# exoplanet-dev/celerite2

Hardware: AMD Instinct MI355X
Metric: float64 GP log-lik+grad/sec at N=4096 J=8, batched (higher is better)
Workload: dtype f64; 1 GPU; configs[2]: batch of 65536 independent GPs (65536 per GPU), N=4096, J=8 (sum of 4 SHO terms), forward + reverse-mode grad, inputs resident in HBM; global_batch=65536, batch_per_gpu=65536, N=4096, J=8, parallelism=batch-sharded x1, all-gather of log-liks, failed_factorizations=0, clock_prewarm_steps=0

## Files before the change

### celerite2_amd/csrc/c2_dispatch.hpp

```cpp
#pragma once

#define C2_OPTIONS(X)                                                                                                                 \
  X(lanes, "C2_LANES", 0, 's', "lane mapping of the fused log-likelihood kernels: 8 (a group of lanes per series), 4 (four lanes per series, two columns per lane, J = 8), 2 (two lanes per series, J = 8), 1 (one lane per series); unset: by batch size", "profiles/r02_lane_mappings.md") \
  X(lanes1_min_batch_fwd, "C2_LANES1_MIN_BATCH_FWD", 24576, 't', "forward log-likelihood: one lane per series from this many series up (widths 8, 6, 4, 2)", "N = 4096, J = 8: 3.3 vs 4.1 ms at 24576 series, 6.7 vs 10.4 ms at 65536 (profiles/r02_lane_mappings.md)") \
  X(lanes1_min_batch_grad, "C2_LANES1_MIN_BATCH_GRAD", 24576, 't', "log-likelihood + gradient: one lane per series from this many series up (widths 8, 4, 2)", "15.7 vs 16.0 ms at 24576 series, 28.2 vs 41.8 ms at 65536 (profiles/r02_lane_mappings.md)") \
  X(lanes1_min_batch_grad_j6, "C2_LANES1_MIN_BATCH_GRAD_J6", 32768, 't', "the same at width 6 (rows of 48 bytes: no aligned 128-byte runs)", "18.5 vs 20.7 ms at 32768 series, 17.2 vs 15.8 ms at 24576") \
  X(lanes2_min_batch_fwd, "C2_LANES2_MIN_BATCH_FWD", 16385, 't', "forward log-likelihood, J = 8: two lanes per series from this many series up ...", "N = 4096: 2.38 - 2.57 vs 2.25 - 2.43 ms at 16384 series (two columns per lane: one wavefront per SIMD there), 2.59 vs 3.69 at 20480 (one lane), 2.76 vs 3.70 at 24576, 3.37 vs 3.84 at 32768 (profiles/r04_two_lanes.md)") \
  X(lanes2_min_batch_grad, "C2_LANES2_MIN_BATCH_GRAD", 16385, 't', "log-likelihood + gradient, J = 8: two lanes per series from this many series up ...", "11.0 vs 14.6 ms at 18432 series (8 lanes: a third round of wavefronts), 11.4 vs 14.4 at 20480, 12.2 - 12.5 vs 15.2 at 24576; 10.25 vs 10.11 at 16384, 10.17 vs 9.65 at 14336 (8 lanes, reverse sweep by the backward recursion; profiles/r04_two_lanes.md)") \
  X(lanes2_max_batch, "C2_LANES2_MAX_BATCH", 32768, 't', "... up to this many (32 series per wavefront: one wavefront per SIMD)", "14.9 - 16.0 vs 16.2 - 17.2 ms at 32768 series (box to box), 27.5 vs 19.4 at 34816 (profiles/r04_two_lanes.md)") \
  X(loglik_back, "C2_LOGLIK_BACK", 1, 's', "log-likelihood + gradient on the group mappings (up to eight lanes per series): reverse sweep by the BACKWARD recursion from recorded W rows instead of replaying the forward steps; 0 keeps the replay (A/B runs)", "profiles/r04_back8.md") \
  X(lanes4_min_batch, "C2_LANES4_MIN_BATCH", 16384, 't', "forward log-likelihood, J = 8: two columns per lane from this many series up", "14-15 % faster from 16384 series, equal at 8192 (profiles/r01_lanes4.md)") \
  X(lanes4_min_batch_grad, "C2_LANES4_MIN_BATCH_GRAD", 9216, 't', "log-likelihood + gradient, J = 8: four lanes per series (two columns per lane, scaled frame; c2_loglik_q4.hip) from this many series up ...", "N = 4096: 4.99 vs 4.52 ms at 8192 series (8 lanes: one wavefront per SIMD there), 6.10 vs 6.43 at 9216, 6.21 vs 6.60 at 10240, 6.94 vs 7.36 at 12288 (profiles/r05_four_lanes.md)") \
  X(lanes4_max_batch_grad, "C2_LANES4_MAX_BATCH_GRAD", 16384, 't', "... up to this many (one wavefront per SIMD; the two-lane pair takes over beyond)", "8.39 ms at 16384 series against 9.7 on eight lanes at two wavefronts per SIMD (profiles/r05_four_lanes.md)") \
  X(loglik_q4_lines, "C2_LOGLIK_Q4_LINES", 0, 's', "the four-lane gradient pair moves the rows of U, V, bU, bV as aligned 128-byte lines of eight series through LDS tiles (1) or 64 bytes of sixteen series at a time (0); unset: lines from C2_Q4_LINES_MIN_BATCH series", "profiles/r05_four_lanes.md") \
  X(q4_lines_min_batch, "C2_Q4_LINES_MIN_BATCH", 11264, 't', "... that batch size", "N = 4096, lines vs rows: 6.53 vs 6.55 ms at 10240 series, 6.68 vs 6.87 at 12288, 8.20 vs 9.00 at 14336, 8.39 vs 8.96 at 16384; 5.53 vs 5.29 at 8192 (profiles/r05_four_lanes.md)") \
  X(timepar, "C2_TIMEPAR", 0, 's', "forward log-likelihood / factor (widths 4, 2) and the single-rhs solves parallel along TIME: 1 forces, 0 disables; unset: by a cost model (C2_TIMEPAR_ELEMENTS_BIAS) / for small batches of long series", "tools/onepass_grid.py, profiles/r05_onepass.md") \
  X(timepar_min_rows, "C2_TIMEPAR_MIN_ROWS", 1536, 't', "shortest series the time-parallel single-rhs SOLVES take when the batch is not a handful (B * J > 512)", "a handful of series from 384 / 704 / 1024 rows at widths 2 / 4 / 8 (profiles/r02_timepar.md)") \
  X(timepar_max_batch_x_width, "C2_TIMEPAR_MAX_BATCH_X_WIDTH", 8192, 't', "largest B * J the time-parallel single-rhs solves take", "linear in the batch beyond one wavefront per SIMD (profiles/r02_timepar.md)") \
  X(timepar_elements_bias, "C2_TIMEPAR_ELEMENTS_BIAS", 100, 't', "forward log-likelihood (widths 8, 4, 2) and factor (widths 4, 2): the time-parallel forms on chunk elements are taken when their modelled time x this / 100 is below the row-by-row kernel's (the model: use_timepar in c2_loglik.hip; 50 favours them, 200 the row-by-row kernels)", "width 4, 1024 series: log-likelihood 0.044 ms up to 1024 rows, 0.109 at 4096 (row by row 0.22 us per row); factor 0.09 / 0.25 ms; 4096 x 4096: 0.38 vs 0.88 and 0.82 vs 1.02 ms; 8192 x 1024: 0.28 vs 0.24 (tools/onepass_grid.py, profiles/r05_onepass.md)") \
  X(timepar_grad, "C2_TIMEPAR_GRAD", 0, 's', "log-likelihood GRADIENT (and factor_rev) parallel along time, widths 1 .. 8: 1 forces, 0 disables; unset: small batches of long series", "tools/timepar_grad_time.py, profiles/r02_timepar_grad.md") \
  X(timepar_grad_min_rows, "C2_TIMEPAR_GRAD_MIN_ROWS", 1024, 't', "shortest series the time-parallel gradient takes at widths 7, 8 beyond a handful of series (768 at widths 3 .. 6, 512 at 1, 2; 256 for at most 4096 chunks)", "one series draws level at ~400 / ~600 / ~800 rows at J = 2 / 4, 6 / 8 (tools/timepar_grad_time.py)") \
  X(timepar_grad_min_rows_handful, "C2_TIMEPAR_GRAD_MIN_ROWS_HANDFUL", 384, 't', "shortest series the time-parallel gradient takes for a handful of series (at most 4096 chunks of 64 rows; they run with 16-row chunks)", "round 5 (the row-by-row pair in the scaled frame), one series, J = 8: 0.336 vs 0.276 ms row by row at 256 rows, 0.381 vs 0.376 at 384, 0.430 vs 0.476 at 512, 0.87 vs 3.25 at 4096 (tools/crossovers.py)") \
  X(timepar_grad_max_chunks, "C2_TIMEPAR_GRAD_MAX_CHUNKS", 32768, 't', "largest number of 64-row chunks (B * ceil(N / 64)) the time-parallel gradient takes", "1024 x 4096 at J = 4: 3.6 vs 3.0 ms row by row") \
  X(timepar_cond_limit, "C2_TIMEPAR_COND_LIMIT", 0, 't', "if > 0: largest conditioning kappa = max a_n / d_n for which the result of the time-parallel gradient stands; beyond it the row-by-row kernels recompute the batch behind the device-side gate (0, the default: no limit)", "rounding moves ANY float64 evaluation by c eps kappa^2 of the largest gradient entry: the oracle itself c = 0.4 (against its own extended-precision evaluation), the row-by-row kernels ~0.05, the time-parallel form ~0.01 and 0.6 in the worst draw of 9000 -- typically the closer of the two to the oracle, hence no limit by default (tools/kappa_sweep.py, tools/verify_words.py, profiles/r03_timepar_verification.md)") \
  X(verify_fallback, "C2_VERIFY_FALLBACK", 1, 's', "0 (diagnostics only): keep the result of a time-parallel form whatever its device-side verification says", "tools/verify_words.py") \
  X(factor_iter, "C2_FACTOR_ITER", 0, 's', "factor by Newton iterations on the chunk start states: 1 forces, 0 disables; unset: from 2048 rows and at most 32768 chunks (widths 4, 2: from 32768 / 131072 rows)", "tools/factor_iter_time.py: 4096 rows 1.21 -> 0.76 ms, 1e5 rows 29.5 -> 1.0 ms at J = 8") \
  X(factor_scan8, "C2_FACTOR_SCAN8", 1, 's', "width 8: the chunk start states of that form EXACT from the scanned chunk elements (up-sweep + down-sweep of the tree, then ONE pass) instead of Newton iterations on them; 0: the iterations", "tools/kernel_breakdown.sh factor 1 4096 8: eight iterations 513 us (profiles/r06_scan8.md)") \
  X(tpg_rows, "C2_TPG_ROWS", 0, 's', "chunk length of the time-parallel gradient / Newton factor / chunk-map solves: 16, 32 or 64; unset: 16 up to 4096 rows and 32 beyond for at most 4096 chunks of 64 rows, else 64 (the log-likelihood gradient: 32 up to 9216 chunks of 64 rows)", "one series of 4096 rows 1.33 -> 1.03 -> 0.73 ms (64 -> 32 -> 16 rows), 1e5 rows 1.68 -> 1.25 ms with 32") \
  X(tpg_rows16_max_rows, "C2_TPG_ROWS16_MAX_ROWS", 4096, 't', "longest series that takes 16-row chunks", "chains of more than 256 chunks cost accuracy first (9000 rows: 1.3e-11 vs 4e-12), then time") \
  X(dropin_long_rows, "C2_DROPIN_LONG_ROWS", 512, 't', "shortest series factor + S and factor_rev take in their time-parallel form (at least 128)", "tools/bench_ops.py, J = 8: factor_rev 1 x 512 0.38 -> 0.15 ms, 512 x 4096 3.0 -> 1.6 ms") \
  X(long_min_rows, "C2_LONG_MIN_ROWS", 512, 't', "shortest series the chunk-map solves (with F / several right-hand sides) and the long-series reverse sweeps take (at least 128)", "1 x 4096 + F 0.60 -> 0.06 ms, 64 x 1024 0.13 -> 0.05 ms (tools/bench_ops.py)") \
  X(rev_long, "C2_REV_LONG", 0, 's', "the four reverse sweeps as opposite sweep + per-row pass: 1 forces, 0 disables; unset: small batches of long series", "one series of 1e5 rows, J = 8: solve_lower_rev 18.3 -> 0.15 ms (profiles/r02_long_series_rocprof.md)") \
  X(scan_min_rows, "C2_SCAN_MIN_ROWS", 1024, 't', "shortest series the chunked products (c2_scan.hip) take on batches of at most 128 series (at least 256)", "1 x 4096 0.60 -> 0.08 ms, 64 x 4096 0.63 -> 0.15 ms; 1024 x 2048 would lose (0.36 -> 1.01 ms)") \
  X(scan_min_chunk, "C2_SCAN_MIN_CHUNK", 0, 's', "chunk length of the chunked products (at least 64); unset: the power of two next to 0.5 sqrt(N)", "one series, J = 8: 20000 rows 0.79 -> 0.16 ms, 1e5 rows 0.80 -> 0.32 ms") \
  X(solve_chunk_col_ms, "C2_SOLVE_CHUNK_COL_MS", 0.05, 't', "cost model of the chunk-map solves: fixed cost (ms) of one right-hand side", "64 x 4096: 0.07 ms, 512 x 4096: 0.24 ms (tools/bench_ops.py)") \
  X(solve_chunk_ms, "C2_SOLVE_CHUNK_MS", 6e-6, 't', "... cost (ms) per 64-row chunk and right-hand side", "same measurement") \
  X(solve_row_us, "C2_SOLVE_ROW_US", 0.15, 't', "... against the row-by-row sweep: microseconds per row whatever the batch", "4096 rows: 0.63 ms with one right-hand side") \
  X(solve_row_rhs_us, "C2_SOLVE_ROW_RHS_US", 0.025, 't', "... plus microseconds per row and right-hand side", "4096 rows: 1.29 ms with 8 right-hand sides") \
  X(sweep_cols, "C2_SWEEP_COLS", 1, 's', "0: forward sweeps with 9 .. 32 right-hand sides at J = 8 (no workspace) on the lanes-over-rhs kernel (16 / 32 lanes per series) instead of eight lanes per series with several columns per lane and Y / Z in groups of four rows; 2: the second column slice of a reverse sweep with 17 .. 24 right-hand sides keeps two columns per lane instead of one (A/B runs)", "B = 8192, N = 4096: profiles/r04_nrhs_scan.md; one column per lane for the narrow slice: solve_lower_rev at 17 / 20 / 24 right-hand sides 25.2 / 23.5 / 23.5 -> 20.0 / 20.9 / 20.4 ms (profiles/r05_nrhs_scan.md)") \
  X(solve_cols, "C2_SOLVE_COLS", 0, 's', "solve_lower / solve_upper without workspace as chunk maps with lanes over the right-hand sides (every column in the same three launches; J <= 16): 1 forces, 0 disables; unset: 16 and more right-hand sides on small batches, by the cost model of solve_cols_shape", "1 x 4096 with 1024 right-hand sides: profiles/r04_large_nrhs.md") \
  X(solve_cols_min_rows, "C2_SOLVE_COLS_MIN_ROWS", 512, 't', "shortest series that form takes", "below, a launch is a few hundred steps of 0.26 us: nothing to gain behind three launches") \
  X(mfma, "C2_MFMA", 1, 's', "0: long-series products (J = 16; 16 / 32 / 64 right-hand sides) on the VALU instead of the fp64 matrix cores", "N = 1e7: 3.1 vs 9.2 ms (profiles/r02_ubench_memory_and_mfma.md)") \
  X(kernel_values_tile, "C2_KERNEL_VALUES_TILE", 1, 's', "0: c2_kernel_values with a thread (an exponential and a sincos) per entry instead of 32 x 64 tiles with one sincos per tile row / column and angle addition", "64 x 4096 x 256, four complex terms: 1.04 ms per entry (profiles/r06_predict.md)") \
// ... 49 lines not shown
```

### celerite2_amd/csrc/c2_loglik.hip

```cpp
#include <cstdint>
#include <cstdlib>
#include <type_traits>

#include "c2_loglik_helpers.hpp"
#include "../../include/celerite2_amd.h"
#include "c2_internal.hpp"
#include "c2_launch.hpp"

#ifdef C2_REV_TIMING
__device__ unsigned long long c2_dbg[8];
extern "C" void c2_internal_read_dbg(unsigned long long *out) {
  hipMemcpyFromSymbol(out, HIP_SYMBOL(c2_dbg), sizeof(unsigned long long) * 8);
  unsigned long long z[8] = {0};
  hipMemcpyToSymbol(HIP_SYMBOL(c2_dbg), z, sizeof(z));
}
#endif

namespace c2 {

template <int G>
struct Ckpt {
  static constexpr int W = G + 4;
};

template <int G>
__device__ __forceinline__ void fwd_chain(double p, double u, double v, double an, double yn, const double (&pX)[G],
                                          const double (&uX)[G], double (&SX)[G], double &F, double &w, double &d,
                                          double &z, double &rd, double *xslot, int lane, double *tau_out = nullptr) {
  double wX[G];
  xgather_dpp<G>(w, xslot, lane, wX);
  const double dw = d * w;
  double tau0 = 0.0, tau1 = 0.0;
#pragma unroll
  for (int k = 0; k < G; ++k) {
    const double s = (pX[k] * p) * fma(dw, wX[k], SX[k]);
    SX[k] = s;
    if (k & 1) tau1 = fma(uX[k], s, tau1);
    else tau0 = fma(uX[k], s, tau0);
  }
  const double tau = tau0 + tau1;
  if (tau_out) *tau_out = tau;
  F = p * fma(w, z, F);
  double rd_ = tau * u, rz_ = u * F;
  gsum2<G>(rd_, rz_);
  const double dn = an - rd_;
  const double zn = yn - rz_;
  rd = rcp_nr(dn);
  w = (v - tau) * rd;
  d = dn;
  z = zn;
}

#ifndef C2_FWD_RING
#define C2_FWD_RING 8
#endif
#ifndef C2_FWD_OCC
#define C2_FWD_OCC 1
#endif
#ifndef C2_REV_OCC
#define C2_REV_OCC 1
#endif
#ifndef C2_REV_APARK
#define C2_REV_APARK 1
#endif
template <int G>
struct SymPack {
  static constexpr int PER_STEP = kWave + (G - 1) * (kWave / 2);
  static __device__ __forceinline__ int off(int l, int k) {
    const int b = 31 - __builtin_clz(k), hb = 1 << b;
    const int o = (l & hb) ? (l ^ k) : l;
    const int idx = ((o >> (b + 1)) << b) | (o & (hb - 1));
    return kWave + (k - 1) * (kWave / 2) + idx;
  }
};

// ... 127 lines not shown
  if (b < B) {
    const double xm = fmax(fabs(x[b * x_bs]), fabs(x[b * x_bs + N - 1]));
    for (int k = 0; k < T.Jc; ++k) fast = fast && (fabs(T.dc[(T.batched ? b * T.Jc : 0) + k]) * xm < kSincosFastMax);
  }
  double m = 0.0;
  if (words && (int)threadIdx.x < wpg && wpg * g + threadIdx.x < nwaves) {
    m = __longlong_as_double((long long)words[2 * (wpg * g + threadIdx.x) + 1]);
    if (m != m) m = __builtin_inf();
  }
#pragma unroll
  for (int sft = 1; sft < kWave; sft <<= 1) m = fmax(m, __shfl_xor(m, sft, kWave));
  if (!__all(fast)) m = __builtin_inf();
  if (threadIdx.x == 0) {
    const unsigned long long bits = (unsigned long long)__double_as_longlong(m);
    gate[g] = bits;
    atomicMax(head, bits);
    if (!(m <= kBackwardGuard)) atomicAdd(head + 1, 1ull);
  }
}

template <int G, int R, int C, int MODE, bool PAD, int OCC = C2_FWD_OCC, bool TT = false>
__global__ __launch_bounds__(kWave, OCC) void k_loglik_fwd(int64_t B, int64_t N, int Jrt, const double *__restrict__ t,
                                                         int64_t t_bs, const double *__restrict__ c, int64_t c_bs,
                                                         const double *__restrict__ a,
                                                         const double *__restrict__ U,
                                                         const double *__restrict__ V,
                                                         const double *__restrict__ y, double *__restrict__ ll,
                                                         int32_t *__restrict__ flag, double *__restrict__ ckpt,
                                                         int64_t nseg, double *__restrict__ Wst,
                                                         double2 *__restrict__ DZst,
                                                         const unsigned long long *__restrict__ gate,
                                                         const unsigned long long *__restrict__ segguard = nullptr,
                                                         TermsArgs8 T8 = TermsArgs8{},
                                                         const unsigned long long *__restrict__ tgate = nullptr) {
  if (gate_closed(gate, (int64_t)blockIdx.x * (kWave / G))) return;
  static_assert(!TT || (G >= 2 && G <= 8 && !PAD && MODE != 2), "coefficient-level form: full groups of two to eight lanes");
  if constexpr (TT) { if (!tt_group_open(tgate, (int64_t)blockIdx.x * (kWave / G))) return; }
  constexpr bool CKPT = MODE == 1, FACTOR = MODE == 2, REC = MODE != 0;
  static_assert(!CKPT || R % C == 0, "block length must be a multiple of the checkpoint interval");
  constexpr int SPW = kWave / G;
  constexpr int NV = (R + G - 1) / G;
  __shared__ __attribute__((aligned(16))) double xs[3][kWave];
  __shared__ __attribute__((aligned(16))) double sin_[2][3][SPW][R];
  __shared__ __attribute__((aligned(16))) double2 sout[SPW][R];
  const int J = PAD ? Jrt : G;
  const Geo<G> L(B, J);
  const int lane = L.lane, j = L.j, grp = L.lane / G;
  const bool act = PAD ? L.act : true;
  const int64_t ot = (int64_t)L.sl * t_bs, on = (int64_t)L.sl * N, oj = (int64_t)L.sl * N * J + L.jj;
  const double *tb = t + L.b0 * t_bs + ot, *ab = a + L.b0 * N + on, *yb = y + L.b0 * N + on;
  const double *Ub = U + L.b0 * N * J + oj, *Vb = V + L.b0 * N * J + oj;
  const double cj = act ? c[L.b * c_bs + j] : 0.0;
  LaneTerm lt;
  if constexpr (TT) lt.load(T8, L.b, j, G);
  double *ckw = CKPT ? ckpt + (size_t)blockIdx.x * (nseg + (segguard != nullptr ? 1 : 0)) * CkptRec<G>::DOUBLES : nullptr;
  int soff[G];
  soff[0] = lane;
#pragma unroll
  for (int k = 1; k < G; ++k) soff[k] = SymPack<G>::off(lane, k);
  const bool wrec = CKPT && Wst != nullptr;
  double *wst = FACTOR ? Wst + L.b0 * N * J + oj : nullptr;
  double *wrp = wrec ? Wst + (size_t)blockIdx.x * N * kWave + lane : nullptr;
  double2 *dzst = CKPT ? DZst + L.b0 * N + on : nullptr;
  double *dst = FACTOR ? reinterpret_cast<double *>(DZst) + L.b0 * N + on : nullptr;
  const bool stw = PAD ? (L.valid && act) : true;

  double SX[G];
#pragma unroll
  for (int k = 0; k < G; ++k) SX[k] = 0.0;
  double d = 1.0;
  double rd = 1.0;
  double w = 0.0;
  double z = 0.0;
  double F = 0.0;
  double prod = 1.0;
  int eacc = 0;
  double quad = 0.0;
  int32_t fl = 0;

  double vt[NV], va[NV], vy[NV];
  auto vload = [&](int64_t nb) {
#pragma unroll
    for (int m = 0; m < NV; ++m) {
      int64_t row = nb + m * G + j;
      row = (row < N) ? row : N - 1;
      vt[m] = tb[row]; va[m] = ab[row]; vy[m] = yb[row];
    }
  };
  auto vstage = [&](int q) {
#pragma unroll
    for (int m = 0; m < NV; ++m) {
      const int idx = m * G + j;
      if (G * NV == R || idx < R) {
        sin_[q][0][grp][idx] = vt[m]; sin_[q][1][grp][idx] = va[m]; sin_[q][2][grp][idx] = vy[m];
      }
    }
  };
  vload(0); vstage(0);
  vload(R); vstage(1);
  vload(2 * R);

  constexpr int RR = R < C2_FWD_RING ? R : C2_FWD_RING;
  double ru[RR], rv[RR];
  const double *up = Ub, *vp = Vb;
  auto load_row = [&](int r, int ahead, int64_t n, bool clamp) {
    if constexpr (!TT) {
      int64_t o = ahead;
      if (clamp && n >= N) o -= n - (N - 1);
      ru[r] = act ? up[o * J] : 0.0; rv[r] = act ? vp[o * J] : 0.0;
    }
  };
#pragma unroll
  for (int r = 0; r < RR; ++r) load_row(r, r, r, true);

  const bool sparse = wrec && !(__longlong_as_double((long long)segguard[2 * blockIdx.x]) > kBackwardGuard);
  lds_order();
  double tnext = sin_[0][0][grp][0];
  double pc = 1.0, uc = ru[0];
  double vcur = 0.0;
  if constexpr (TT) lt.uv(tnext, uc, vcur);
  double pXc[G], uXc[G];
  xs[0][lane] = pc; xs[1][lane] = uc;
  lds_order();
  xgather_lds<G>(xs[0], lane, pXc);
  xgather_lds<G>(xs[1], lane, uXc);
  lds_order();

  auto block = [&](int64_t n0, int q, auto checked_tag) {
    constexpr bool CHECKED = decltype(checked_tag)::value;
#pragma unroll
    for (int r = 0; r < R; ++r) {
      const int64_t n = n0 + r;
      if (!CHECKED || n < N) {
        if (CKPT && (r % C == 1 % C)) {
          const int64_t m = (n - 1) / C;
          if (!sparse || (m % kAnchor == 0 && m > 0))
            ckpt_store<G>(ckw + m * CkptRec<G>::DOUBLES, lane, soff, SX, F, w);
        }
        const double tn = tnext, yn = sin_[q][2][grp][r];
        const double an = TT ? sin_[q][1][grp][r] + lt.A0 : sin_[q][1][grp][r];
        const double tn1 = (r + 1 < R) ? sin_[q][0][grp][r + 1] : sin_[q ^ 1][0][grp][0];
        const int rn = (r + 1) % R;
        double v, un1;
        if constexpr (TT) {
          v = vcur;
          lt.uv(tn1, un1, vcur);
        } else {
          v = rv[r % RR]; un1 = ru[rn % RR];
        }
        const double pn1 = exp_decay(cj * (tn - tn1));
        double pXn[G], uXn[G];
        xs[0][lane] = pn1; xs[1][lane] = un1;
        lds_order();
        xgather_lds<G>(xs[0], lane, pXn);
        xgather_lds<G>(xs[1], lane, uXn);
        lds_order();
        fwd_chain<G>(pc, uc, v, an, yn, pXc, uXc, SX, F, w, d, z, rd, xs[2], lane);
        if (REC) {
          if (FACTOR && stw && (((fl == 0) & (d > 0.0)) | (n == 0))) wst[n * J] = w;
          if (CKPT && wrec) wrp[(size_t)n * kWave] = w;
          sout[grp][r] = make_double2(d, z);
        }
        load_row(r % RR, r + RR, n + RR, CHECKED);
        fl = ((fl == 0) & (d <= 0.0)) ? (int32_t)n : fl;
        prod *= d;
        quad = fma(z * z, rd, quad);
        if (r % 2 == 1 || r == R - 1) {
          int e;
          prod = frexp(prod, &e);
          eacc += e;
        }
        tnext = tn1;
        pc = pn1; uc = un1;
#pragma unroll
        for (int k = 0; k < G; ++k) { pXc[k] = pXn[k]; uXc[k] = uXn[k]; }
      }
    }
    lds_order();
    if (REC) {
#pragma unroll
      for (int m = 0; m < NV; ++m) {
        const int idx = m * G + j;
        if ((G * NV == R || idx < R) && (!CHECKED || n0 + idx < N)) {
          if (CKPT) dzst[n0 + idx] = sout[grp][idx];
          else if (fl == 0 || n0 + idx <= fl) dst[n0 + idx] = sout[grp][idx].x;
        }
      }
    }
    vstage(q);
    vload(n0 + 3 * R);
    lds_order();
  };
  int64_t n0 = 0;
  int q = 0;
  auto advance = [&]() { up += R * J; vp += R * J; q ^= 1; };
  for (; n0 + 2 * R <= N; n0 += R) { block(n0, q, std::false_type{}); advance(); }
  for (; n0 < N; n0 += R) { block(n0, q, std::true_type{}); advance(); }

  if (wrec) ckpt_store<G>(ckw + nseg * CkptRec<G>::DOUBLES, lane, soff, SX, F, w);
  if (L.valid && j == 0) {
    flag[L.b] = fl;
    if (!FACTOR) {
      int e;
      prod = frexp(prod, &e);
      const double logdet = log(prod) + (double)(eacc + e) * kLn2;
      ll[L.b] = fl ? -INFINITY : -0.5 * (logdet + (double)N * kLog2Pi) - 0.5 * quad;
    }
  }
}

__device__ __forceinline__ void apark(double x, int &lo, int &hi) {
  asm("v_accvgpr_write_b32 %0, %1" : "=a"(lo) : "v"(__double2loint(x)));
  asm("v_accvgpr_write_b32 %0, %1" : "=a"(hi) : "v"(__double2hiint(x)));
}
__device__ __forceinline__ double afetch(int lo, int hi) {
  int l, h;
  asm("v_accvgpr_read_b32 %0, %1" : "=v"(l) : "a"(lo));
  asm("v_accvgpr_read_b32 %0, %1" : "=v"(h) : "a"(hi));
  return __hiloint2double(h, l);
}

template <int G, int C, bool PAD, bool FR, bool BACK = false, int OCC = C2_REV_OCC, bool TT = false>
__global__ __launch_bounds__(kWave, OCC) void k_loglik_rev(int64_t B, int64_t N, int Jrt, const double *__restrict__ t,
                                                         int64_t t_bs, const double *__restrict__ c, int64_t c_bs,
                                                         const double *__restrict__ U,
                                                         const double *__restrict__ V,
                                                         const double2 *__restrict__ DZst,
                                                         const double *__restrict__ ckpt, int64_t nseg,
                                                         const int32_t *__restrict__ flag, double *__restrict__ bt,
                                                         double *__restrict__ bc, double *__restrict__ ba,
                                                         double *__restrict__ bU, double *__restrict__ bV,
// ... 70 lines not shown
  const double wD = (TT && !lt.re && !lt.odd) ? lt.D : 0.0;
  int vAlo[TT ? C : 1], vAhi[TT ? C : 1];

  int soff[G];
  soff[0] = lane;
#pragma unroll
  for (int k = 1; k < G; ++k) soff[k] = SymPack<G>::off(lane, k);

  double MX[G];
#pragma unroll
  for (int k = 0; k < G; ++k) MX[k] = 0.0;
  double bF = 0.0, carry = 0.0, bcj = 0.0;
  double bVn = 0.0, ban = 0.0, bzn = 0.0;

  double vt[NV];
  double2 vdz[NV];
  double iu[C], iw[C], ibw[FR ? C : 1];
  double cS[G], cF = 0.0, cW = 0.0, tck = 0.0;
  auto load_segment = [&](int64_t k) {
    const int64_t n_lo = 1 + k * C;
    const bool full = n_lo + C <= N;
#pragma unroll
    for (int m = 0; m < NV; ++m) {
      int64_t row = n_lo - 1 + m * G + j;
      row = (row < N) ? row : N - 1;
      vt[m] = tb[row];
      if constexpr (FR) vdz[m] = make_double2(fdb[row], fbdb[row]);
      else vdz[m] = dzb[row];
    }
#pragma unroll
    for (int r = 0; r < C; ++r) {
      const int64_t n = (full || n_lo + r < N) ? n_lo + r : N - 1;
      if constexpr (!TT) iu[r] = act ? Ub[n * J] : 0.0;
      if constexpr (BACK) iw[r] = V[((size_t)blockIdx.x * N + (n - 1)) * kWave + lane];
      else iw[r] = act ? Vb[(n - 1) * J] : 0.0;
      if constexpr (FR) ibw[r] = act ? fbWb[(n - 1) * J] : 0.0;
    }
    if constexpr (FR) {
      const int64_t m = n_lo - 1;
#pragma unroll
      for (int kk = 0; kk < G; ++kk) {
        const int i = j ^ kk;
        cS[kk] = (m >= 1 && act && i < J) ? Scol[m * J * J + i] : 0.0;
      }
      tck = tb[m >= 1 ? m - 1 : 0];
    } else if constexpr (BACK) {
      if ((k + 1) % astep == 0 || k == nseg - 1)
        ckpt_load<G>(ckw + (k + 1) * CkptRec<G>::DOUBLES, lane, soff, cS, cF, cW);
    } else {
      ckpt_load<G>(ckw + k * CkptRec<G>::DOUBLES, lane, soff, cS, cF, cW);
    }
  };

  double carT = tb[N - 1];
  double2 carDZ = FR ? make_double2(fdb[N - 1], fbdb[N - 1]) : dzb[N - 1];
  double carR = rcp_nr(carDZ.x);
  const double wlast = (FR && act) ? Vb[(N - 1) * J] : 0.0, bwlast = (FR && act) ? fbWb[(N - 1) * J] : 0.0;
  if (nseg > 0) load_segment(nseg - 1);
#ifdef C2_REV_TIMING
  unsigned long long tacc[5] = {0, 0, 0, 0, 0}, tlast = 0;
#define C2_TCK(i) do { const unsigned long long tn_ = __builtin_readcyclecounter(); if (i) tacc[i] += tn_ - tlast; tlast = tn_; } while (0)
#else
#define C2_TCK(i)
#endif

  double carS[BACK ? G : 1], carF = 0.0;
  double tref = 0.0, gtop = 1.0, igtop = 1.0;
#pragma unroll
  for (int i = 0; i < (BACK ? G : 1); ++i) carS[i] = 0.0;
// ... 409 lines not shown
    const int JC = T8.Jc, JR = G - 2 * JC;
    const double bcp = dpp_mov<kDppXor1>(bcj);
    if (lt.re) { G8.bar[L.b * JR + j] = sba + accA; G8.bcr[L.b * JR + j] = bcj; }
    else if (!lt.odd) {
      const int64_t o = L.b * JC + ((j - JR) >> 1);
      G8.bac[o] = sba + accA; G8.bbc[o] = accB; G8.bdc[o] = accD; G8.bcc[o] = bcj + bcp;
    }
  } else if (st) { bVb[0] = BACK ? bVn * gtop : bVn; bUb[0] = 0.0; bc[L.b * J + j] = bcj; }
}

}

using namespace c2;

#ifndef C2_CKPT_C
#define C2_CKPT_C 8
#endif
#ifndef C2_FWD_R
#define C2_FWD_R C2_CKPT_C
#endif
#ifndef C2_FWD_R8
#define C2_FWD_R8 16
#endif

static int64_t simd_count();
namespace {
template <int MODE>
int launch_fwd(int64_t B, int64_t N, int64_t J, const double *t, int64_t t_bs, const double *c, int64_t c_bs,
               const double *a, const double *U, const double *V, const double *y, double *ll, int32_t *flag,
               double *ckpt, int64_t nseg, double *Wst, double2 *DZst, hipStream_t s,
               const unsigned long long *gate = nullptr, const unsigned long long *segguard = nullptr, bool occ2 = false) {
  const int G_ = group_size(J);
  const dim3 grid((unsigned)((B * G_ + kWave - 1) / kWave));
  if (MODE == 1 && occ2 && J == 8) {
    hipLaunchKernelGGL((k_loglik_fwd<8, C2_FWD_R8, C2_CKPT_C, (MODE == 1 ? 1 : 0), false, 2>), grid, dim3(kWave), 0, s, B, N, (int)J, t, t_bs, c,
                       c_bs, a, U, V, y, ll, flag, ckpt, nseg, Wst, DZst, gate, segguard);
    return launch_ok();
  }
#define C2_FWD(G, R, C)                                                                                          \
  do {                                                                                                           \
    if (J == G)                                                                                                  \
      hipLaunchKernelGGL((k_loglik_fwd<G, R, C, MODE, false>), grid, dim3(kWave), 0, s, B, N, (int)J, t, t_bs,   \
                         c, c_bs, a, U, V, y, ll, flag, ckpt, nseg, Wst, DZst, gate, segguard);                 \
    else                                                                                                         \
      hipLaunchKernelGGL((k_loglik_fwd<G, R, C, MODE, true>), grid, dim3(kWave), 0, s, B, N, (int)J, t, t_bs,    \
                         c, c_bs, a, U, V, y, ll, flag, ckpt, nseg, Wst, DZst, gate, segguard);                 \
  } while (0)
  switch (G_) {
    case 1: C2_FWD(1, C2_FWD_R, C2_CKPT_C); break;
    case 2: C2_FWD(2, C2_FWD_R, C2_CKPT_C); break;
    case 4: C2_FWD(4, C2_FWD_R, C2_CKPT_C); break;
    case 8: C2_FWD(8, C2_FWD_R8, C2_CKPT_C); break;
    case 16: C2_FWD(16, 8, 4); break;
    default: C2_FWD(32, 4, 2); break;
  }
#undef C2_FWD
  return launch_ok();
}
}

static bool use_lanes4(int64_t B, int64_t J, bool grad) {
  if (J != 8) return false;
  const int forced = opt::has(opt::k_lanes) ? (int)opt::ival(opt::k_lanes) : 0;
  if (forced == 4) return true;
  if (forced == 8 || forced == 1 || forced == 2) return false;
  if (grad) return B >= opt::ival(opt::k_lanes4_min_batch_grad) && B <= opt::ival(opt::k_lanes4_max_batch_grad);
  return B >= opt::ival(opt::k_lanes4_min_batch);
}

static size_t lanes1_gate_words(int64_t B) { return (size_t)((kGateHeadWords + (B + kWave - 1) / kWave + 1) & ~(int64_t)1); }
static bool use_lanes2(int64_t B, int64_t N, int64_t J, bool grad) {
  if (!c2_internal_loglik_k2_ok(B, N, J)) return false;
  const int forced = opt::has(opt::k_lanes) ? (int)opt::ival(opt::k_lanes) : 0;
  if (forced) return forced == 2;
  return B <= opt::ival(opt::k_lanes2_max_batch) &&
         B >= opt::ival(grad ? opt::k_lanes2_min_batch_grad : opt::k_lanes2_min_batch_fwd);
}
static size_t lanes1_record_doubles(int64_t B, int64_t N, int64_t J) {
  return J == 8 ? c2_internal_loglik_t_record_doubles8(B, N)
// ... 153 lines not shown
      rc = keep_first(rc, hipFreeAsync(tmp, s));
      return rc;
    }
    (void)hipGetLastError();
  }
  if (capturing == hipStreamCaptureStatusNone && use_timepar(B, N, J, true)) {
    const size_t nd = c2_internal_loglik_timepar_doubles(B, N, J);
    void *tmp = nullptr;
    if (nd > 0 && c2::temp_alloc(&tmp, (nd + 2) * sizeof(double), s) == hipSuccess) {
      unsigned long long *guard = (unsigned long long *)tmp;
      int rc = c2_internal_loglik_timepar(B, N, J, t, t_bs, c, c_bs, a, U, V, y, ll, flag, (double *)tmp + 2, guard, stream);
      if (rc == C2_OK)
        rc = launch_fwd<0>(B, N, J, t, t_bs, c, c_bs, a, U, V, y, ll, flag, nullptr, 0, nullptr, nullptr, s, guard + 1);
      rc = keep_first(rc, hipFreeAsync(tmp, s));
      return rc;
    }
    (void)hipGetLastError();
  }
  return launch_fwd<0>(B, N, J, t, t_bs, c, c_bs, a, U, V, y, ll, flag, nullptr, 0, nullptr, nullptr, s);
}

static inline int ckpt_interval(int G_) { return G_ <= 8 ? C2_CKPT_C : (G_ == 16 ? 4 : 2); }

struct GradWs {
  size_t ck, w, dz, guard, total;
};
static inline GradWs grad_ws(int64_t B, int64_t N, int64_t J, bool back = false) {
  const int G_ = group_size(J), C_ = ckpt_interval(G_);
  const int64_t nseg = (N - 1 + C_ - 1) / C_;
  GradWs g;
  const size_t waves = ((size_t)B * G_ + kWave - 1) / kWave;
  g.ck = waves * (size_t)(nseg + (back ? 1 : 0)) * ((size_t)kWave + (size_t)(G_ - 1) * (kWave / 2) + 2 * kWave);
  g.ck = (g.ck + 1) & ~(size_t)1;
  g.w = back ? waves * (size_t)N * kWave : 0;
  g.dz = (size_t)B * N * 2;
  g.guard = back ? 2 * waves : 0;
  g.total = g.ck + g.w + g.dz + g.guard;
  return g;
}
static int64_t simd_count() {
  static int64_t n = 0;
  if (n == 0) {
    int dev = 0, cus = 0;
    if (hipGetDevice(&dev) != hipSuccess || hipDeviceGetAttribute(&cus, hipDeviceAttributeMultiprocessorCount, dev) != hipSuccess || cus <= 0)
      cus = 256;
    n = 4 * (int64_t)cus;
  }
  return n;
}
static bool use_back(int64_t N, int64_t J) {
  if (opt::off(opt::k_loglik_back)) return false;
  return group_size(J) <= 8 && N >= 2;
}

size_t c2_internal_factor_scratch_doubles(int64_t B, int64_t N, int64_t J) {
  const size_t n1 = c2_internal_factor_iter_doubles(B, N, J), n2 = c2_internal_timepar_doubles(B, N, J) + 2;
  return ((n1 > n2 ? n1 : n2) + 1) & ~(size_t)1;
}
int c2_internal_factor_fused_ws(int64_t B, int64_t N, int64_t J, const double *t, int64_t t_bs, const double *c,
                                int64_t c_bs, const double *a, const double *U, const double *V, double *d, double *W,
                                int32_t *flag, int allow_timepar, double *scratch, c2_stream_t stream) {
  hipStream_t s = (hipStream_t)stream;
  hipStreamCaptureStatus capturing = hipStreamCaptureStatusNone;
  (void)hipStreamIsCapturing(s, &capturing);
  const bool may_alloc = capturing == hipStreamCaptureStatusNone;
  auto room = [&](size_t nd, void **tmp) {
    if (scratch) { *tmp = scratch; return true; }
// ... 299 lines not shown
}

size_t c2_internal_loglik_g8_tt_doubles(int64_t B, int64_t N, int64_t J) { return grad_ws(B, N, J, true).total; }
int c2_internal_loglik_g8_tt_ok(int64_t B, int64_t N, int64_t J) {
  return (J == 8 || J == 4 || J == 2) && N >= 2 && B >= 1 && (B * J + kWave - 1) / kWave <= simd_count();
}
int c2_internal_loglik_g8_tt_grad(int64_t B, int64_t N, int64_t J, int64_t Jc, int coef_batched, const double *ar, const double *ac,
                                  const double *bc, const double *dc, const double *c, const double *x, int64_t x_bs,
                                  const double *diag, const double *y, double *ll, double *bar, double *bcr, double *bac,
                                  double *bbc, double *bcc, double *bdc, double *bx, double *bdiag, double *by,
                                  int32_t *flag, double *work, unsigned long long *guard, c2_stream_t stream) {
  if (Jc < 0 || 2 * Jc > J || !c2_internal_loglik_g8_tt_ok(B, N, J)) return C2_ERR_UNSUPPORTED;
  hipStream_t s = (hipStream_t)stream;
  constexpr int C_ = C2_CKPT_C;
  const int64_t nseg = (N - 1 + C_ - 1) / C_;
  const GradWs ws = grad_ws(B, N, J, true);
  double *ckpt = work, *Wrec = ckpt + ws.ck;
  double2 *DZst = reinterpret_cast<double2 *>(ckpt + ws.ck + ws.w);
  unsigned long long *segg = reinterpret_cast<unsigned long long *>(ckpt + ws.ck + ws.w + ws.dz);
  const dim3 grid((unsigned)((B * J + kWave - 1) / kWave));
  const TermsArgs8 T{ar, ac, bc, dc, coef_batched, (int)Jc};
  const TermsGrads8 G{bar, bcr, bac, bbc, bcc, bdc};
  unsigned long long *tgate = guard + kGateHeadWords;
  hipLaunchKernelGGL(k_anchor_spans, grid, dim3(256), 0, s, B, N, (int)J, C_, kWave / (int)J, x, x_bs, c, J, segg);
  if (int e = launch_ok()) return e;
  if (int e = hip_check(hipMemsetAsync(guard, 0, 8 * kGateHeadWords, s))) return e;
  hipLaunchKernelGGL(k_tt8_gate, dim3((unsigned)((B + 63) / 64)), dim3(kWave), 0, s, B, N, (int64_t)grid.x, (int)J,
                     (const unsigned long long *)segg, T, x, x_bs, guard, tgate);
  if (int e = launch_ok()) return e;
#define C2_TTG(G_, R_)                                                                                                                \
  do {                                                                                                                                \
    hipLaunchKernelGGL((k_loglik_fwd<G_, R_, C2_CKPT_C, 1, false, 1, true>), grid, dim3(kWave), 0, s, B, N, G_, x, x_bs, \
                       c, J, diag, (const double *)nullptr, (const double *)nullptr, y, ll, flag, ckpt, nseg, Wrec, DZst,             \
                       (const unsigned long long *)nullptr, (const unsigned long long *)segg, T, (const unsigned long long *)tgate);  \
    if (int e = launch_ok()) return e;                                                                                                \
    hipLaunchKernelGGL((k_loglik_rev<G_, C2_CKPT_C, false, false, true, 1, true>), grid, dim3(kWave), 0, s, B, N, G_, x,  \
                       x_bs, c, J, (const double *)nullptr, (const double *)Wrec, (const double2 *)DZst, (const double *)ckpt, nseg,  \
                       (const int32_t *)flag, bx, (double *)nullptr, bdiag, (double *)nullptr, (double *)nullptr, by,                 \
                       (const double *)nullptr, (const double *)nullptr, (const double *)nullptr,                                     \
                       (const unsigned long long *)nullptr, (const unsigned long long *)segg, T, G, (const unsigned long long *)tgate); \
  } while (0)
  if (J == 8) C2_TTG(8, C2_FWD_R8);
  else if (J == 4) C2_TTG(4, C2_FWD_R);
  else C2_TTG(2, C2_FWD_R);
#undef C2_TTG
  return launch_ok();
}
int c2_internal_loglik_g8_tt(int64_t B, int64_t N, int64_t J, int64_t Jc, int coef_batched, const double *ar, const double *ac,
                             const double *bc, const double *dc, const double *c, const double *x, int64_t x_bs,
                             const double *diag, const double *y, double *ll, int32_t *flag, unsigned long long *guard,
                             c2_stream_t stream) {
  if (!(J == 8 || J == 4 || J == 2) || Jc < 0 || 2 * Jc > J || B < 1 || N < 1) return C2_ERR_UNSUPPORTED;
  hipStream_t s = (hipStream_t)stream;
  const dim3 grid((unsigned)((B * J + kWave - 1) / kWave));
  const TermsArgs8 T{ar, ac, bc, dc, coef_batched, (int)Jc};
  unsigned long long *tgate = guard + kGateHeadWords;
  if (int e = hip_check(hipMemsetAsync(guard, 0, 8 * kGateHeadWords, s))) return e;
  hipLaunchKernelGGL(k_tt8_gate, dim3((unsigned)((B + 63) / 64)), dim3(kWave), 0, s, B, N, (int64_t)grid.x, (int)J,
                     (const unsigned long long *)nullptr, T, x, x_bs, guard, tgate);
  if (int e = launch_ok()) return e;
#define C2_TTF(G_, R_)                                                                                                                \
  hipLaunchKernelGGL((k_loglik_fwd<G_, R_, C2_CKPT_C, 0, false, 1, true>), grid, dim3(kWave), 0, s, B, N, G_, x, x_bs, c, \
                     J, diag, (const double *)nullptr, (const double *)nullptr, y, ll, flag, (double *)nullptr, (int64_t)0,           \
                     (double *)nullptr, (double2 *)nullptr, (const unsigned long long *)nullptr, (const unsigned long long *)nullptr, \
                     T, (const unsigned long long *)tgate)
  if (J == 8) C2_TTF(8, C2_FWD_R8);
  else if (J == 4) C2_TTF(4, C2_FWD_R);
// ... 43 lines not shown
```

Measured before the change: 2.374 million GP/s.

## Run eight-lane gradient forward pass in scaled frame between anchors, record W in pairs

Inside the backward guard, the forward log-likelihood pass on the group lane mappings now works in a frame rescaled at periodic anchors. This drops the per-row decay product and its LDS gather and exchange, and replaces them with one scaling factor gathered through DPP. The recorded W rows are also stored and read as double2 pairs, which halves the number of record transactions in both the forward and the reverse kernels. The cost is extra rescaling at anchors and a new numerical path that can be switched off with an option. The one-lane mapping selected at this batch size may not go through this kernel.

```diff
diff --git a/celerite2_amd/csrc/c2_dispatch.hpp b/celerite2_amd/csrc/c2_dispatch.hpp
--- a/celerite2_amd/csrc/c2_dispatch.hpp
+++ b/celerite2_amd/csrc/c2_dispatch.hpp
@@ -9,6 +9,7 @@
   X(lanes2_min_batch_grad, "C2_LANES2_MIN_BATCH_GRAD", 16385, 't', "log-likelihood + gradient, J = 8: two lanes per series from this many series up ...", "11.0 vs 14.6 ms at 18432 series (8 lanes: a third round of wavefronts), 11.4 vs 14.4 at 20480, 12.2 - 12.5 vs 15.2 at 24576; 10.25 vs 10.11 at 16384, 10.17 vs 9.65 at 14336 (8 lanes, reverse sweep by the backward recursion; profiles/r04_two_lanes.md)") \
   X(lanes2_max_batch, "C2_LANES2_MAX_BATCH", 32768, 't', "... up to this many (32 series per wavefront: one wavefront per SIMD)", "14.9 - 16.0 vs 16.2 - 17.2 ms at 32768 series (box to box), 27.5 vs 19.4 at 34816 (profiles/r04_two_lanes.md)") \
   X(loglik_back, "C2_LOGLIK_BACK", 1, 's', "log-likelihood + gradient on the group mappings (up to eight lanes per series): reverse sweep by the BACKWARD recursion from recorded W rows instead of replaying the forward steps; 0 keeps the replay (A/B runs)", "profiles/r04_back8.md") \
+  X(loglik_fwd_scaled, "C2_LOGLIK_FWD_SCALED", 1, 't', "log-likelihood + gradient on the group mappings (up to eight lanes per series): 1 (the default), the forward pass of a wavefront within the backward guard runs in the scaled frame between anchors (no decay products per row); 0 keeps the unscaled loop for every wavefront (A/B runs; both sides in tests/test_gpu_eight_lane_frame.py)", "profiles/eight_lane_forward_frame.md") \
   X(lanes4_min_batch, "C2_LANES4_MIN_BATCH", 16384, 't', "forward log-likelihood, J = 8: two columns per lane from this many series up", "14-15 % faster from 16384 series, equal at 8192 (profiles/r01_lanes4.md)") \
   X(lanes4_min_batch_grad, "C2_LANES4_MIN_BATCH_GRAD", 9216, 't', "log-likelihood + gradient, J = 8: four lanes per series (two columns per lane, scaled frame; c2_loglik_q4.hip) from this many series up ...", "N = 4096: 4.99 vs 4.52 ms at 8192 series (8 lanes: one wavefront per SIMD there), 6.10 vs 6.43 at 9216, 6.21 vs 6.60 at 10240, 6.94 vs 7.36 at 12288 (profiles/r05_four_lanes.md)") \
   X(lanes4_max_batch_grad, "C2_LANES4_MAX_BATCH_GRAD", 16384, 't', "... up to this many (one wavefront per SIMD; the two-lane pair takes over beyond)", "8.39 ms at 16384 series against 9.7 on eight lanes at two wavefronts per SIMD (profiles/r05_four_lanes.md)") \
diff --git a/celerite2_amd/csrc/c2_loglik.hip b/celerite2_amd/csrc/c2_loglik.hip
--- a/celerite2_amd/csrc/c2_loglik.hip
+++ b/celerite2_amd/csrc/c2_loglik.hip
@@ -41,6 +41,33 @@
   const double tau = tau0 + tau1;
   if (tau_out) *tau_out = tau;
   F = p * fma(w, z, F);
+  double rd_ = tau * u, rz_ = u * F;
+  gsum2<G>(rd_, rz_);
+  const double dn = an - rd_;
+  const double zn = yn - rz_;
+  rd = rcp_nr(dn);
+  w = (v - tau) * rd;
+  d = dn;
+  z = zn;
+}
+
+template <int G>
+__device__ __forceinline__ void fwd_chain_scaled(double u, double v, double an, double yn, const double (&uX)[G],
+                                                 double (&SX)[G], double &F, double &w, double &d, double &z, double &rd,
+                                                 double *xslot, int lane) {
+  double wX[G];
+  xgather_dpp<G>(w, xslot, lane, wX);
+  const double dw = d * w;
+  double tau0 = 0.0, tau1 = 0.0;
+#pragma unroll
+  for (int k = 0; k < G; ++k) {
+    const double s = fma(dw, wX[k], SX[k]);
+    SX[k] = s;
+    if (k & 1) tau1 = fma(uX[k], s, tau1);
+    else tau0 = fma(uX[k], s, tau0);
+  }
+  const double tau = tau0 + tau1;
+  F = fma(w, z, F);
   double rd_ = tau * u, rz_ = u * F;
   gsum2<G>(rd_, rz_);
   const double dn = an - rd_;
@@ -234,7 +261,8 @@
                                                          const unsigned long long *__restrict__ gate,
                                                          const unsigned long long *__restrict__ segguard = nullptr,
                                                          TermsArgs8 T8 = TermsArgs8{},
-                                                         const unsigned long long *__restrict__ tgate = nullptr) {
+                                                         const unsigned long long *__restrict__ tgate = nullptr,
+                                                         int fscaled = 1) {
   if (gate_closed(gate, (int64_t)blockIdx.x * (kWave / G))) return;
   static_assert(!TT || (G >= 2 && G <= 8 && !PAD && MODE != 2), "coefficient-level form: full groups of two to eight lanes");
   if constexpr (TT) { if (!tt_group_open(tgate, (int64_t)blockIdx.x * (kWave / G))) return; }
@@ -262,7 +290,9 @@
   for (int k = 1; k < G; ++k) soff[k] = SymPack<G>::off(lane, k);
   const bool wrec = CKPT && Wst != nullptr;
   double *wst = FACTOR ? Wst + L.b0 * N * J + oj : nullptr;
-  double *wrp = wrec ? Wst + (size_t)blockIdx.x * N * kWave + lane : nullptr;
+  static_assert(!CKPT || R % 2 == 0, "rows are recorded in pairs: a block starts at an even row");
+  double2 *wrp = wrec ? reinterpret_cast<double2 *>(Wst) + (size_t)blockIdx.x * ((N + 1) >> 1) * kWave + lane : nullptr;
+  double whold = 0.0;
   double2 *dzst = CKPT ? DZst + L.b0 * N + on : nullptr;
   double *dst = FACTOR ? reinterpret_cast<double *>(DZst) + L.b0 * N + on : nullptr;
   const bool stw = PAD ? (L.valid && act) : true;
@@ -316,6 +346,9 @@
   for (int r = 0; r < RR; ++r) load_row(r, r, r, true);
 
   const bool sparse = wrec && !(__longlong_as_double((long long)segguard[2 * blockIdx.x]) > kBackwardGuard);
+  constexpr bool FRAME = CKPT && G <= 8 && OCC == 1;
+  const bool scaled = FRAME && sparse && fscaled != 0;
+  double tref = 0.0, gc = 1.0, igc = 1.0;
   lds_order();
   double tnext = sin_[0][0][grp][0];
   double pc = 1.0, uc = ru[0];
@@ -328,8 +361,9 @@
   xgather_lds<G>(xs[1], lane, uXc);
   lds_order();
 
-  auto block = [&](int64_t n0, int q, auto checked_tag) {
+  auto block = [&](int64_t n0, int q, auto checked_tag, auto scaled_tag) {
     constexpr bool CHECKED = decltype(checked_tag)::value;
+    constexpr bool SC = decltype(scaled_tag)::value;
 #pragma unroll
     for (int r = 0; r < R; ++r) {
       const int64_t n = n0 + r;
@@ -350,17 +384,41 @@
         } else {
           v = rv[r % RR]; un1 = ru[rn % RR];
         }
-        const double pn1 = exp_decay(cj * (tn - tn1));
-        double pXn[G], uXn[G];
-        xs[0][lane] = pn1; xs[1][lane] = un1;
-        lds_order();
-        xgather_lds<G>(xs[0], lane, pXn);
-        xgather_lds<G>(xs[1], lane, uXn);
-        lds_order();
-        fwd_chain<G>(pc, uc, v, an, yn, pXc, uXc, SX, F, w, d, z, rd, xs[2], lane);
+        double pn1 = 1.0, gn1 = 1.0, ign1 = 1.0, wout;
+        double pXn[SC ? 1 : G], uXn[G];
+        if constexpr (SC) {
+          const bool anchor = (r % C == 0) && n > 0 && (n / C) % kAnchor == 0;
+          if (anchor) tref = tn;
+          gn1 = exp_decay(cj * (tref - tn1));
+          ign1 = rcp_nr(gn1);
+          un1 *= gn1;
+          xgather_dpp<G>(un1, xs[1], lane, uXn);
+          fwd_chain_scaled<G>(uc, v * igc, an, yn, uXc, SX, F, w, d, z, rd, xs[2], lane);
+          wout = w * gc;
+          if (anchor) {
+            double gX[G];
+            xgather_dpp<G>(gc, xs[2], lane, gX);
+#pragma unroll
+            for (int k = 0; k < G; ++k) SX[k] *= gX[k] * gc;
+            F *= gc;
+            w = wout;
+          }
+        } else {
+          pn1 = exp_decay(cj * (tn - tn1));
+          xs[0][lane] = pn1; xs[1][lane] = un1;
+          lds_order();
+          xgather_lds<G>(xs[0], lane, pXn);
+          xgather_lds<G>(xs[1], lane, uXn);
+          lds_order();
+          fwd_chain<G>(pc, uc, v, an, yn, pXc, uXc, SX, F, w, d, z, rd, xs[2], lane);
+          wout = w;
+        }
         if (REC) {
           if (FACTOR && stw && (((fl == 0) & (d > 0.0)) | (n == 0))) wst[n * J] = w;
-          if (CKPT && wrec) wrp[(size_t)n * kWave] = w;
+          if (CKPT && wrec) {
+            if (r % 2 == 0) whold = wout;
+            else wrp[(size_t)(n >> 1) * kWave] = make_double2(whold, wout);
+          }
           sout[grp][r] = make_double2(d, z);
         }
         load_row(r % RR, r + RR, n + RR, CHECKED);
@@ -374,8 +432,14 @@
         }
         tnext = tn1;
         pc = pn1; uc = un1;
-#pragma unroll
-        for (int k = 0; k < G; ++k) { pXc[k] = pXn[k]; uXc[k] = uXn[k]; }
+        if constexpr (SC) {
+          gc = gn1; igc = ign1;
+#pragma unroll
+          for (int k = 0; k < G; ++k) uXc[k] = uXn[k];
+        } else {
+#pragma unroll
+          for (int k = 0; k < G; ++k) { pXc[k] = pXn[k]; uXc[k] = uXn[k]; }
+        }
       }
     }
     lds_order();
@@ -396,9 +460,23 @@
   int64_t n0 = 0;
   int q = 0;
   auto advance = [&]() { up += R * J; vp += R * J; q ^= 1; };
-  for (; n0 + 2 * R <= N; n0 += R) { block(n0, q, std::false_type{}); advance(); }
-  for (; n0 < N; n0 += R) { block(n0, q, std::true_type{}); advance(); }
-
+  if constexpr (FRAME) {
+    if (scaled) {
+      tref = tnext;
+      for (; n0 + 2 * R <= N; n0 += R) { block(n0, q, std::false_type{}, std::true_type{}); advance(); }
+      for (; n0 < N; n0 += R) { block(n0, q, std::true_type{}, std::true_type{}); advance(); }
+      double gX[G];
+      xgather_dpp<G>(gc, xs[2], lane, gX);
+#pragma unroll
+      for (int k = 0; k < G; ++k) SX[k] *= gX[k] * gc;
+      F *= gc;
+      w *= gc;
+    }
+  }
+  for (; n0 + 2 * R <= N; n0 += R) { block(n0, q, std::false_type{}, std::false_type{}); advance(); }
+  for (; n0 < N; n0 += R) { block(n0, q, std::true_type{}, std::false_type{}); advance(); }
+
+  if (wrec && (N & 1)) reinterpret_cast<double *>(wrp + (size_t)(N >> 1) * kWave)[0] = whold;
   if (wrec) ckpt_store<G>(ckw + nseg * CkptRec<G>::DOUBLES, lane, soff, SX, F, w);
   if (L.valid && j == 0) {
     flag[L.b] = fl;
@@ -535,9 +613,20 @@
     for (int r = 0; r < C; ++r) {
       const int64_t n = (full || n_lo + r < N) ? n_lo + r : N - 1;
       if constexpr (!TT) iu[r] = act ? Ub[n * J] : 0.0;
-      if constexpr (BACK) iw[r] = V[((size_t)blockIdx.x * N + (n - 1)) * kWave + lane];
-      else iw[r] = act ? Vb[(n - 1) * J] : 0.0;
+      if constexpr (!BACK) iw[r] = act ? Vb[(n - 1) * J] : 0.0;
       if constexpr (FR) ibw[r] = act ? fbWb[(n - 1) * J] : 0.0;
+    }
+    if constexpr (BACK) {
+      static_assert(!BACK || C % 2 == 0, "the W record holds pairs of rows");
+      const int64_t np = (N + 1) >> 1;
+      const double2 *wrec2 = reinterpret_cast<const double2 *>(V) + (size_t)blockIdx.x * np * kWave + lane;
+#pragma unroll
+      for (int i = 0; i < C / 2; ++i) {
+        int64_t pm = k * (C / 2) + i;
+        if (!full && pm >= np) pm = np - 1;
+        const double2 wp = wrec2[pm * kWave];
+        iw[2 * i] = wp.x; iw[2 * i + 1] = wp.y;
+      }
     }
     if constexpr (FR) {
       const int64_t m = n_lo - 1;
@@ -1013,19 +1102,23 @@
                const unsigned long long *gate = nullptr, const unsigned long long *segguard = nullptr, bool occ2 = false) {
   const int G_ = group_size(J);
   const dim3 grid((unsigned)((B * G_ + kWave - 1) / kWave));
+  const int fsc = opt::ival(opt::k_loglik_fwd_scaled) != 0;
   if (MODE == 1 && occ2 && J == 8) {
     hipLaunchKernelGGL((k_loglik_fwd<8, C2_FWD_R8, C2_CKPT_C, (MODE == 1 ? 1 : 0), false, 2>), grid, dim3(kWave), 0, s, B, N, (int)J, t, t_bs, c,
-                       c_bs, a, U, V, y, ll, flag, ckpt, nseg, Wst, DZst, gate, segguard);
+                       c_bs, a, U, V, y, ll, flag, ckpt, nseg, Wst, DZst, gate, segguard, TermsArgs8{},
+                       (const unsigned long long *)nullptr, fsc);
     return launch_ok();
   }
 #define C2_FWD(G, R, C)                                                                                          \
   do {                                                                                                           \
     if (J == G)                                                                                                  \
       hipLaunchKernelGGL((k_loglik_fwd<G, R, C, MODE, false>), grid, dim3(kWave), 0, s, B, N, (int)J, t, t_bs,   \
-                         c, c_bs, a, U, V, y, ll, flag, ckpt, nseg, Wst, DZst, gate, segguard);                 \
+                         c, c_bs, a, U, V, y, ll, flag, ckpt, nseg, Wst, DZst, gate, segguard, TermsArgs8{},    \
+                         (const unsigned long long *)nullptr, fsc);                                             \
     else                                                                                                         \
       hipLaunchKernelGGL((k_loglik_fwd<G, R, C, MODE, true>), grid, dim3(kWave), 0, s, B, N, (int)J, t, t_bs,    \
-                         c, c_bs, a, U, V, y, ll, flag, ckpt, nseg, Wst, DZst, gate, segguard);                 \
+                         c, c_bs, a, U, V, y, ll, flag, ckpt, nseg, Wst, DZst, gate, segguard, TermsArgs8{},    \
+                         (const unsigned long long *)nullptr, fsc);                                             \
   } while (0)
   switch (G_) {
     case 1: C2_FWD(1, C2_FWD_R, C2_CKPT_C); break;
@@ -1245,7 +1338,7 @@
   const size_t waves = ((size_t)B * G_ + kWave - 1) / kWave;
   g.ck = waves * (size_t)(nseg + (back ? 1 : 0)) * ((size_t)kWave + (size_t)(G_ - 1) * (kWave / 2) + 2 * kWave);
   g.ck = (g.ck + 1) & ~(size_t)1;
-  g.w = back ? waves * (size_t)N * kWave : 0;
+  g.w = back ? waves * (size_t)((N + 1) / 2) * 2 * kWave : 0;
   g.dz = (size_t)B * N * 2;
   g.guard = back ? 2 * waves : 0;
   g.total = g.ck + g.w + g.dz + g.guard;
@@ -1611,7 +1704,8 @@
   do {                                                                                                                                \
     hipLaunchKernelGGL((k_loglik_fwd<G_, R_, C2_CKPT_C, 1, false, 1, true>), grid, dim3(kWave), 0, s, B, N, G_, x, x_bs, \
                        c, J, diag, (const double *)nullptr, (const double *)nullptr, y, ll, flag, ckpt, nseg, Wrec, DZst,             \
-                       (const unsigned long long *)nullptr, (const unsigned long long *)segg, T, (const unsigned long long *)tgate);  \
+                       (const unsigned long long *)nullptr, (const unsigned long long *)segg, T, (const unsigned long long *)tgate,  \
+                       (int)(opt::ival(opt::k_loglik_fwd_scaled) != 0));                                                              \
     if (int e = launch_ok()) return e;                                                                                                \
     hipLaunchKernelGGL((k_loglik_rev<G_, C2_CKPT_C, false, false, true, 1, true>), grid, dim3(kWave), 0, s, B, N, G_, x,  \
                        x_bs, c, J, (const double *)nullptr, (const double *)Wrec, (const double2 *)DZst, (const double *)ckpt, nseg,  \
```

Result: slower. 2.305 million GP/s (-2.9%).
